# YangHai-1218/RADet

Measured on AMD Instinct MI355X. Metric: images/sec train-step, r50_ycbv_pbr 640x480 bs=4/GPU, higher is better.
Workload: dtype f32

## Files before the change

include/radet_hip.h:

```cpp
#ifndef RADET_HIP_H
#define RADET_HIP_H
#include <stdint.h>

#ifdef __cplusplus
extern "C" {
#endif


typedef struct RadetConvDesc {
    const float* w;
    const float* bias;
    const float* bn_gamma;
    const float* bn_beta;
    const float* bn_mean;
    const float* bn_var;
    float* wf;
    float* wft;
    float* bias_f;
    const float* dwf_slabs;
    const float* dbias_partials;
    float* dw;
    float* dbias;
    float* dgamma;
    float* dbeta;
// ... 192 lines not shown
                             void* yp1, float* stats1, float* partial_ws1, int B, int C, int groups, float eps, int relu,
                             const int* seg_desc, int nseg, void* stream);
int radet_gn_relu_bwd_p(const float* dy, const float* z, const float* stats, const float* gamma, const float* beta,
                        float* dz, void* dzp, float* dgamma, float* dbeta, float* partial_ws, int B, int C, int groups,
                        int relu, const int* seg_desc, int nseg, void* stream);
int radet_nchw_to_nhwc(const float* x, float* y, int B, int C, int H, int W, void* stream);
int radet_nhwc_to_nchw(const float* x, float* y, int B, int C, int H, int W, void* stream);

int radet_head_loss_ws_ints(int R);
int radet_head_loss(const float* cls, const float* reg_u, const float* iou, const float* scales,
                    const float* gt_boxes, const int64_t* gt_labels, const int* gt_off, const int64_t* p2g,
                    const float* pw, const int* level_desc, int nlvl, int B, int num_classes, float alpha,
                    float gamma, float loss_bbox_weight, float giou_eps, const float* grad_scale, float* losses,
                    float* dcls, int dcls_ld, float* dreg_u, int dreg_ld, float* diou, int diou_ld, float* dscales,
                    int64_t* labels_out, float* bbox_targets_out, int flags, int* ws, void* stream);
int radet_scale_relu(const float* reg_u, const float* scales, float* out, const int* level_desc, int nlvl, int B,
                     void* stream);

size_t radet_decode_ws_bytes(int B, int nlvl, int nms_pre);
int radet_decode_candidates(const float* cls, const float* reg_u, const float* iou, const float* scales,
                            const int* level_desc, int nlvl, int B, int num_classes, float score_thr, int nms_pre,
                            const float* img_hw , const float* scale_factor ,
                            float* cand_boxes, float* cand_scores, float* cand_ctr, int64_t* cand_labels,
                            int* cand_count, void* ws, void* stream);

size_t radet_nms_ws_bytes(int B, int cap);
int radet_nms(const float* boxes, const float* cluster_scores, const float* vote_scores, const int64_t* labels,
              const int* counts, int B, int cap, int mode, float iou_thr, int iou_enable, float sigma, int max_out,
              float* out_boxes, float* out_scores, int64_t* out_labels, int* out_count, int64_t* aux0, int64_t* aux1,
              void* ws, void* stream);
// ... 169 lines not shown
```

radet_amd/_lib.py:

```python
import ctypes as C
import os

_HERE = os.path.dirname(os.path.abspath(__file__))
LIB_PATH = os.path.join(_HERE, os.environ.get("RADET_LIB", "libradet_hip.so"))

_p = C.c_void_p
_i = C.c_int
_f = C.c_float
_sz = C.c_size_t


class RadetConvDesc(C.Structure):
    _fields_ = [("w", _p), ("bias", _p), ("bn_gamma", _p), ("bn_beta", _p), ("bn_mean", _p), ("bn_var", _p),
                ("wf", _p), ("wft", _p), ("bias_f", _p), ("dwf_slabs", _p), ("dbias_partials", _p),
                ("dw", _p), ("dbias", _p), ("dgamma", _p), ("dbeta", _p),
                ("cout", _i), ("cin", _i), ("kh", _i), ("kw", _i), ("nsplit", _i), ("eps", _f),
                ("wft_ld", _i), ("wft_off", _i), ("w16", _i), ("w_amax", _p), ("wfq", _p), ("w_l1", _p), ("bias_amax", _p),
                ("w_l1t", _p)]


class RadetScales(C.Structure):
    _fields_ = [("x_amax", _p), ("w_amax", _p), ("y_amax", _p), ("x1_amax", _p), ("w1_amax", _p), ("y1_amax", _p),
                ("yq", _p), ("yq_amax", _p), ("x_true_amax", _p), ("w_l1", _p), ("bias_amax", _p), ("addend_amax", _p)]

# ... 45 lines not shown
    "radet_stem_wgrad": (_i, [_p, _p, _p, _p, _i, _i, _i, _i, _p]),
    "radet_gn_workspace_floats": (_i, [_i, _p, _i]),
    "radet_gn_relu_fwd": (_i, [_p, _p, _p, _p, _p, _p, _i, _i, _i, _f, _i, _p, _i, _p]),
    "radet_gn_relu_fwd_pair": (_i, [_p] * 12 + [_i, _i, _i, _f, _i, _p, _i, _p]),
    "radet_gn_relu_fwd_pair_h": (_i, [_p] * 12 + [_i, _i, _i, _f, _i, _p, _i, _p]),
    "radet_gn_relu_bwd": (_i, [_p, _p, _p, _p, _p, _p, _p, _p, _p, _i, _i, _i, _i, _p, _i, _p]),
    "radet_upsample_add": (_i, [_p, _p, _i, _i, _i, _i, _i, _i, _p]),
    "radet_upsample_add_bwd": (_i, [_p, _p, _i, _i, _i, _i, _i, _i, _p]),
    "radet_relu_bwd": (_i, [_p, _p, _p, _p, _sz, _p]),
    "radet_nchw_to_nhwc": (_i, [_p, _p, _i, _i, _i, _i, _p]),
    "radet_nhwc_to_nchw": (_i, [_p, _p, _i, _i, _i, _i, _p]),
    "radet_head_loss_ws_ints": (_i, [_i]),
    "radet_head_loss": (_i, [_p, _p, _p, _p, _p, _p, _p, _p, _p, _p, _i, _i, _i, _f, _f, _f, _f, _p, _p, _p, _i, _p,
                             _i, _p, _i, _p, _p, _p, _i, _p, _p]),
    "radet_scale_relu": (_i, [_p, _p, _p, _p, _i, _i, _p]),
    "radet_decode_ws_bytes": (_sz, [_i, _i, _i]),
    "radet_decode_candidates": (_i, [_p, _p, _p, _p, _p, _i, _i, _i, _f, _i, _p, _p, _p, _p, _p, _p, _p, _p, _p]),
    "radet_nms_ws_bytes": (_sz, [_i, _i]),
    "radet_nms": (_i, [_p, _p, _p, _p, _p, _i, _i, _i, _f, _i, _f, _i, _p, _p, _p, _p, _p, _p, _p, _p]),
    "radet_assign_ws_bytes": (_sz, [_i, _i]),
    "radet_assign_points": (_i, [_p, _p, _p, _i, _i, _p, _i, _p, _p, _i, _i, _i, _i, _f, _p, _p, _p, _p, _p]),
    "radet_assign_points_f": (_i, [_p, _p, _p, _i, _i, _p, _i, _p, _p, _i, _i, _i, _i, _f, _p, _p, _p, _p, _p]),
    "radet_resize_linear_u8": (_i, [_p, _p, _p, _p, _i, _i, _i, _p]),
    "radet_resize_linear_u8_window": (_i, [_p, _p, _p, _p, _i, _i, _i, _p]),
    "radet_resize_linear_u8_src_window": (_i, [_p, _p, _p, _p, _i, _i, _i, _p]),
    "radet_resize_linear_f": (_i, [_p, _p, _p, _p, _i, _i, _i, _p]),
    "radet_warp_affine_u8": (_i, [_p, _sz, _p, _sz, _p, _i, _i, _i, _p]),
    "radet_gaussian_blur9_u8": (_i, [_p, _p, _p, _p, _p, _i, _i, _p]),
    "radet_sobel_edge": (_i, [_p, _p, _p, _p, _p, _i, _i, _p]),
    "radet_stem_conv_bn_relu_h": (_i, [_p, _p, _p, _p, _i, _i, _i, _p]),
# ... 108 lines not shown
```

radet_amd/csrc/tape_thunks.c:

```c
#include <stdint.h>
#include <stddef.h>
#include <string.h>
#include "radet_hip.h"

static float f32(uint64_t w) { uint32_t u = (uint32_t)w; float f; memcpy(&f, &u, 4); return f; }

static int t_radet_absmax(const uint64_t* a) { return radet_absmax((void*)(uintptr_t)a[0], (size_t)a[1], (void*)(uintptr_t)a[2], (void*)(uintptr_t)a[3]); }
static int t_radet_adamw_step(const uint64_t* a) { return radet_adamw_step((void*)(uintptr_t)a[0], (void*)(uintptr_t)a[1], (void*)(uintptr_t)a[2], (void*)(uintptr_t)a[3], (size_t)a[4], f32(a[5]), f32(a[6]), f32(a[7]), f32(a[8]), f32(a[9]), (int)(int64_t)a[10], f32(a[11]), f32(a[12]), (void*)(uintptr_t)a[13], (int)(int64_t)a[14], (void*)(uintptr_t)a[15], (void*)(uintptr_t)a[16]); }
static int t_radet_amax_slot_words(const uint64_t* a) { (void)a; return radet_amax_slot_words(); }
static int t_radet_assign_points(const uint64_t* a) { return radet_assign_points((void*)(uintptr_t)a[0], (void*)(uintptr_t)a[1], (void*)(uintptr_t)a[2], (int)(int64_t)a[3], (int)(int64_t)a[4], (void*)(uintptr_t)a[5], (int)(int64_t)a[6], (void*)(uintptr_t)a[7], (void*)(uintptr_t)a[8], (int)(int64_t)a[9], (int)(int64_t)a[10], (int)(int64_t)a[11], (int)(int64_t)a[12], f32(a[13]), (void*)(uintptr_t)a[14], (void*)(uintptr_t)a[15], (void*)(uintptr_t)a[16], (void*)(uintptr_t)a[17], (void*)(uintptr_t)a[18]); }
static int t_radet_assign_points_f(const uint64_t* a) { return radet_assign_points_f((void*)(uintptr_t)a[0], (void*)(uintptr_t)a[1], (void*)(uintptr_t)a[2], (int)(int64_t)a[3], (int)(int64_t)a[4], (void*)(uintptr_t)a[5], (int)(int64_t)a[6], (void*)(uintptr_t)a[7], (void*)(uintptr_t)a[8], (int)(int64_t)a[9], (int)(int64_t)a[10], (int)(int64_t)a[11], (int)(int64_t)a[12], f32(a[13]), (void*)(uintptr_t)a[14], (void*)(uintptr_t)a[15], (void*)(uintptr_t)a[16], (void*)(uintptr_t)a[17], (void*)(uintptr_t)a[18]); }
static int t_radet_augment_box(const uint64_t* a) { return radet_augment_box((void*)(uintptr_t)a[0], (void*)(uintptr_t)a[1], (void*)(uintptr_t)a[2], (size_t)a[3], (int)(int64_t)a[4], (int)(int64_t)a[5], (int)(int64_t)a[6], (void*)(uintptr_t)a[7]); }
static int t_radet_augment_finish(const uint64_t* a) { return radet_augment_finish((void*)(uintptr_t)a[0], (void*)(uintptr_t)a[1], (void*)(uintptr_t)a[2], (void*)(uintptr_t)a[3], (int)(int64_t)a[4], (int)(int64_t)a[5], (int)(int64_t)a[6], f32(a[7]), f32(a[8]), f32(a[9]), f32(a[10]), f32(a[11]), f32(a[12]), (void*)(uintptr_t)a[13]); }
static int t_radet_augment_hsv_noise(const uint64_t* a) { return radet_augment_hsv_noise((void*)(uintptr_t)a[0], (void*)(uintptr_t)a[1], (void*)(uintptr_t)a[2], (int)(int64_t)a[3], (int)(int64_t)a[4], (void*)(uintptr_t)a[5]); }
static int t_radet_augment_merge_hblur(const uint64_t* a) { return radet_augment_merge_hblur((void*)(uintptr_t)a[0], (void*)(uintptr_t)a[1], (void*)(uintptr_t)a[2], (void*)(uintptr_t)a[3], (int)(int64_t)a[4], (int)(int64_t)a[5], (int)(int64_t)a[6], (void*)(uintptr_t)a[7]); }
static int t_radet_augment_sharp(const uint64_t* a) { return radet_augment_sharp((void*)(uintptr_t)a[0], (void*)(uintptr_t)a[1], (void*)(uintptr_t)a[2], (void*)(uintptr_t)a[3], (int)(int64_t)a[4], (int)(int64_t)a[5], (void*)(uintptr_t)a[6]); }
static int t_radet_augment_vblur(const uint64_t* a) { return radet_augment_vblur((void*)(uintptr_t)a[0], (void*)(uintptr_t)a[1], (void*)(uintptr_t)a[2], (int)(int64_t)a[3], (int)(int64_t)a[4], (int)(int64_t)a[5], (void*)(uintptr_t)a[6]); }
static int t_radet_bbox_overlaps(const uint64_t* a) { return radet_bbox_overlaps((void*)(uintptr_t)a[0], (void*)(uintptr_t)a[1], (void*)(uintptr_t)a[2], (int)(int64_t)a[3], (int)(int64_t)a[4], (int)(int64_t)a[5], (int)(int64_t)a[6], (int)(int64_t)a[7], f32(a[8]), (void*)(uintptr_t)a[9]); }
static int t_radet_bce_logits_loss(const uint64_t* a) { return radet_bce_logits_loss((void*)(uintptr_t)a[0], (void*)(uintptr_t)a[1], (void*)(uintptr_t)a[2], (int)(int64_t)a[3], (size_t)a[4], (int)(int64_t)a[5], (void*)(uintptr_t)a[6], f32(a[7]), (void*)(uintptr_t)a[8], (void*)(uintptr_t)a[9]); }
static int t_radet_bce_logits_loss_bwd(const uint64_t* a) { return radet_bce_logits_loss_bwd((void*)(uintptr_t)a[0], (void*)(uintptr_t)a[1], (void*)(uintptr_t)a[2], (int)(int64_t)a[3], (size_t)a[4], (int)(int64_t)a[5], (void*)(uintptr_t)a[6], (void*)(uintptr_t)a[7], (void*)(uintptr_t)a[8], f32(a[9]), (void*)(uintptr_t)a[10], (void*)(uintptr_t)a[11]); }
static int t_radet_build_gather_table(const uint64_t* a) { return radet_build_gather_table((void*)(uintptr_t)a[0], (int)(int64_t)a[1], (int)(int64_t)a[2], (int)(int64_t)a[3], (int)(int64_t)a[4], (int)(int64_t)a[5], (int)(int64_t)a[6], (int)(int64_t)a[7], (void*)(uintptr_t)a[8], (int)(int64_t)a[9], (void*)(uintptr_t)a[10]); }
static int t_radet_coco_accumulate(const uint64_t* a) { return radet_coco_accumulate((void*)(uintptr_t)a[0], (void*)(uintptr_t)a[1], (void*)(uintptr_t)a[2], (void*)(uintptr_t)a[3], (void*)(uintptr_t)a[4], (void*)(uintptr_t)a[5], (void*)(uintptr_t)a[6], (void*)(uintptr_t)a[7], (int)(int64_t)a[8], (int)(int64_t)a[9], (int)(int64_t)a[10], (int)(int64_t)a[11], (int)(int64_t)a[12], (void*)(uintptr_t)a[13], (void*)(uintptr_t)a[14], (void*)(uintptr_t)a[15], (void*)(uintptr_t)a[16]); }
static int t_radet_coco_match(const uint64_t* a) { return radet_coco_match((void*)(uintptr_t)a[0], (void*)(uintptr_t)a[1], (void*)(uintptr_t)a[2], (void*)(uintptr_t)a[3], (void*)(uintptr_t)a[4], (void*)(uintptr_t)a[5], (int)(int64_t)a[6], (int)(int64_t)a[7], (void*)(uintptr_t)a[8], (int)(int64_t)a[9], (void*)(uintptr_t)a[10], (int)(int64_t)a[11], (void*)(uintptr_t)a[12], (void*)(uintptr_t)a[13], (void*)(uintptr_t)a[14], (void*)(uintptr_t)a[15], (void*)(uintptr_t)a[16]); }
static int t_radet_conv2d_igemm(const uint64_t* a) { return radet_conv2d_igemm((void*)(uintptr_t)a[0], (void*)(uintptr_t)a[1], (void*)(uintptr_t)a[2], (void*)(uintptr_t)a[3], (void*)(uintptr_t)a[4], (void*)(uintptr_t)a[5], (void*)(uintptr_t)a[6], (int)(int64_t)a[7], (int)(int64_t)a[8], (int)(int64_t)a[9], (int)(int64_t)a[10], (int)(int64_t)a[11], (int)(int64_t)a[12], (int)(int64_t)a[13], (void*)(uintptr_t)a[14], (size_t)a[15], (void*)(uintptr_t)a[16]); }
// ... 45 lines not shown
static int t_radet_mask_transform_src_window(const uint64_t* a) { return radet_mask_transform_src_window((void*)(uintptr_t)a[0], (void*)(uintptr_t)a[1], (void*)(uintptr_t)a[2], (void*)(uintptr_t)a[3], (int)(int64_t)a[4], (int)(int64_t)a[5], (int)(int64_t)a[6], (int)(int64_t)a[7], (int)(int64_t)a[8], (int)(int64_t)a[9], (void*)(uintptr_t)a[10]); }
static int t_radet_mask_transform_window(const uint64_t* a) { return radet_mask_transform_window((void*)(uintptr_t)a[0], (void*)(uintptr_t)a[1], (void*)(uintptr_t)a[2], (void*)(uintptr_t)a[3], (int)(int64_t)a[4], (int)(int64_t)a[5], (int)(int64_t)a[6], (int)(int64_t)a[7], (int)(int64_t)a[8], (int)(int64_t)a[9], (void*)(uintptr_t)a[10]); }
static int t_radet_maxpool3x3s2(const uint64_t* a) { return radet_maxpool3x3s2((void*)(uintptr_t)a[0], (void*)(uintptr_t)a[1], (int)(int64_t)a[2], (int)(int64_t)a[3], (int)(int64_t)a[4], (int)(int64_t)a[5], (void*)(uintptr_t)a[6]); }
static int t_radet_maxpool3x3s2_a(const uint64_t* a) { return radet_maxpool3x3s2_a((void*)(uintptr_t)a[0], (void*)(uintptr_t)a[1], (int)(int64_t)a[2], (int)(int64_t)a[3], (int)(int64_t)a[4], (int)(int64_t)a[5], (void*)(uintptr_t)a[6], (void*)(uintptr_t)a[7]); }
static int t_radet_maxpool3x3s2_bwd_relu(const uint64_t* a) { return radet_maxpool3x3s2_bwd_relu((void*)(uintptr_t)a[0], (void*)(uintptr_t)a[1], (void*)(uintptr_t)a[2], (int)(int64_t)a[3], (int)(int64_t)a[4], (int)(int64_t)a[5], (int)(int64_t)a[6], (void*)(uintptr_t)a[7]); }
static int t_radet_maxpool3x3s2_h(const uint64_t* a) { return radet_maxpool3x3s2_h((void*)(uintptr_t)a[0], (void*)(uintptr_t)a[1], (int)(int64_t)a[2], (int)(int64_t)a[3], (int)(int64_t)a[4], (int)(int64_t)a[5], (void*)(uintptr_t)a[6]); }
static int t_radet_maxpool3x3s2_q(const uint64_t* a) { return radet_maxpool3x3s2_q((void*)(uintptr_t)a[0], (void*)(uintptr_t)a[1], (int)(int64_t)a[2], (int)(int64_t)a[3], (int)(int64_t)a[4], (int)(int64_t)a[5], (void*)(uintptr_t)a[6], (void*)(uintptr_t)a[7], (void*)(uintptr_t)a[8], (void*)(uintptr_t)a[9], (void*)(uintptr_t)a[10]); }
static int t_radet_mbd(const uint64_t* a) { return radet_mbd((void*)(uintptr_t)a[0], (void*)(uintptr_t)a[1], (int)(int64_t)a[2], (void*)(uintptr_t)a[3], (void*)(uintptr_t)a[4], f32(a[5]), (int)(int64_t)a[6], (int)(int64_t)a[7], (void*)(uintptr_t)a[8], (size_t)a[9], (void*)(uintptr_t)a[10], (void*)(uintptr_t)a[11]); }
static int t_radet_merge_pairs(const uint64_t* a) { return radet_merge_pairs((void*)(uintptr_t)a[0], (void*)(uintptr_t)a[1], (size_t)a[2], (int)(int64_t)a[3], (int)(int64_t)a[4], (void*)(uintptr_t)a[5], (void*)(uintptr_t)a[6]); }
static int t_radet_merge_planes(const uint64_t* a) { return radet_merge_planes((void*)(uintptr_t)a[0], (void*)(uintptr_t)a[1], (size_t)a[2], (int)(int64_t)a[3], (int)(int64_t)a[4], (void*)(uintptr_t)a[5]); }
static int t_radet_nchw_to_nhwc(const uint64_t* a) { return radet_nchw_to_nhwc((void*)(uintptr_t)a[0], (void*)(uintptr_t)a[1], (int)(int64_t)a[2], (int)(int64_t)a[3], (int)(int64_t)a[4], (int)(int64_t)a[5], (void*)(uintptr_t)a[6]); }
static int t_radet_nhwc_to_nchw(const uint64_t* a) { return radet_nhwc_to_nchw((void*)(uintptr_t)a[0], (void*)(uintptr_t)a[1], (int)(int64_t)a[2], (int)(int64_t)a[3], (int)(int64_t)a[4], (int)(int64_t)a[5], (void*)(uintptr_t)a[6]); }
static int t_radet_nms(const uint64_t* a) { return radet_nms((void*)(uintptr_t)a[0], (void*)(uintptr_t)a[1], (void*)(uintptr_t)a[2], (void*)(uintptr_t)a[3], (void*)(uintptr_t)a[4], (int)(int64_t)a[5], (int)(int64_t)a[6], (int)(int64_t)a[7], f32(a[8]), (int)(int64_t)a[9], f32(a[10]), (int)(int64_t)a[11], (void*)(uintptr_t)a[12], (void*)(uintptr_t)a[13], (void*)(uintptr_t)a[14], (void*)(uintptr_t)a[15], (void*)(uintptr_t)a[16], (void*)(uintptr_t)a[17], (void*)(uintptr_t)a[18], (void*)(uintptr_t)a[19]); }
static int t_radet_paste_maps(const uint64_t* a) { return radet_paste_maps((void*)(uintptr_t)a[0], (size_t)a[1], (int)(int64_t)a[2], (void*)(uintptr_t)a[3], (int)(int64_t)a[4], (int)(int64_t)a[5], (int)(int64_t)a[6], (void*)(uintptr_t)a[7], (void*)(uintptr_t)a[8]); }
static int t_radet_pred3x3_patch(const uint64_t* a) { return radet_pred3x3_patch((void*)(uintptr_t)a[0], (int)(int64_t)a[1], (void*)(uintptr_t)a[2], (int)(int64_t)a[3], (void*)(uintptr_t)a[4], (void*)(uintptr_t)a[5], (void*)(uintptr_t)a[6], (int)(int64_t)a[7], (void*)(uintptr_t)a[8], (void*)(uintptr_t)a[9], (void*)(uintptr_t)a[10], (int)(int64_t)a[11], (void*)(uintptr_t)a[12]); }
static int t_radet_preprocess_frames(const uint64_t* a) { return radet_preprocess_frames((void*)(uintptr_t)a[0], (int)(int64_t)a[1], (int)(int64_t)a[2], (int)(int64_t)a[3], f32(a[4]), f32(a[5]), f32(a[6]), f32(a[7]), f32(a[8]), f32(a[9]), (void*)(uintptr_t)a[10], (void*)(uintptr_t)a[11]); }
static int t_radet_relu_bwd(const uint64_t* a) { return radet_relu_bwd((void*)(uintptr_t)a[0], (void*)(uintptr_t)a[1], (void*)(uintptr_t)a[2], (void*)(uintptr_t)a[3], (size_t)a[4], (void*)(uintptr_t)a[5]); }
static int t_radet_relu_bwd_a(const uint64_t* a) { return radet_relu_bwd_a((void*)(uintptr_t)a[0], (void*)(uintptr_t)a[1], (void*)(uintptr_t)a[2], (void*)(uintptr_t)a[3], (size_t)a[4], (void*)(uintptr_t)a[5], (void*)(uintptr_t)a[6]); }
static int t_radet_relu_bwd_h(const uint64_t* a) { return radet_relu_bwd_h((void*)(uintptr_t)a[0], (void*)(uintptr_t)a[1], (void*)(uintptr_t)a[2], (void*)(uintptr_t)a[3], (size_t)a[4], (void*)(uintptr_t)a[5]); }
static int t_radet_resize_linear_f(const uint64_t* a) { return radet_resize_linear_f((void*)(uintptr_t)a[0], (void*)(uintptr_t)a[1], (void*)(uintptr_t)a[2], (void*)(uintptr_t)a[3], (int)(int64_t)a[4], (int)(int64_t)a[5], (int)(int64_t)a[6], (void*)(uintptr_t)a[7]); }
static int t_radet_resize_linear_u8(const uint64_t* a) { return radet_resize_linear_u8((void*)(uintptr_t)a[0], (void*)(uintptr_t)a[1], (void*)(uintptr_t)a[2], (void*)(uintptr_t)a[3], (int)(int64_t)a[4], (int)(int64_t)a[5], (int)(int64_t)a[6], (void*)(uintptr_t)a[7]); }
static int t_radet_resize_linear_u8_src_window(const uint64_t* a) { return radet_resize_linear_u8_src_window((void*)(uintptr_t)a[0], (void*)(uintptr_t)a[1], (void*)(uintptr_t)a[2], (void*)(uintptr_t)a[3], (int)(int64_t)a[4], (int)(int64_t)a[5], (int)(int64_t)a[6], (void*)(uintptr_t)a[7]); }
static int t_radet_resize_linear_u8_window(const uint64_t* a) { return radet_resize_linear_u8_window((void*)(uintptr_t)a[0], (void*)(uintptr_t)a[1], (void*)(uintptr_t)a[2], (void*)(uintptr_t)a[3], (int)(int64_t)a[4], (int)(int64_t)a[5], (int)(int64_t)a[6], (void*)(uintptr_t)a[7]); }
static int t_radet_rle_masks(const uint64_t* a) { return radet_rle_masks((void*)(uintptr_t)a[0], (int)(int64_t)a[1], (void*)(uintptr_t)a[2], (int)(int64_t)a[3], (void*)(uintptr_t)a[4], (int)(int64_t)a[5], (void*)(uintptr_t)a[6], (void*)(uintptr_t)a[7], (int)(int64_t)a[8], (int)(int64_t)a[9], (int)(int64_t)a[10], (int)(int64_t)a[11], (int)(int64_t)a[12], (void*)(uintptr_t)a[13]); }
static int t_radet_rle_masks_src_window(const uint64_t* a) { return radet_rle_masks_src_window((void*)(uintptr_t)a[0], (int)(int64_t)a[1], (void*)(uintptr_t)a[2], (int)(int64_t)a[3], (void*)(uintptr_t)a[4], (void*)(uintptr_t)a[5], (int)(int64_t)a[6], (void*)(uintptr_t)a[7], (void*)(uintptr_t)a[8], (int)(int64_t)a[9], (int)(int64_t)a[10], (int)(int64_t)a[11], (void*)(uintptr_t)a[12]); }
static int t_radet_rle_masks_window(const uint64_t* a) { return radet_rle_masks_window((void*)(uintptr_t)a[0], (int)(int64_t)a[1], (void*)(uintptr_t)a[2], (int)(int64_t)a[3], (void*)(uintptr_t)a[4], (void*)(uintptr_t)a[5], (int)(int64_t)a[6], (void*)(uintptr_t)a[7], (void*)(uintptr_t)a[8], (int)(int64_t)a[9], (int)(int64_t)a[10], (int)(int64_t)a[11], (void*)(uintptr_t)a[12]); }
static int t_radet_scale_relu(const uint64_t* a) { return radet_scale_relu((void*)(uintptr_t)a[0], (void*)(uintptr_t)a[1], (void*)(uintptr_t)a[2], (void*)(uintptr_t)a[3], (int)(int64_t)a[4], (int)(int64_t)a[5], (void*)(uintptr_t)a[6]); }
static int t_radet_sigmoid_focal_loss(const uint64_t* a) { return radet_sigmoid_focal_loss((void*)(uintptr_t)a[0], (void*)(uintptr_t)a[1], (void*)(uintptr_t)a[2], (int)(int64_t)a[3], (size_t)a[4], (int)(int64_t)a[5], f32(a[6]), f32(a[7]), (void*)(uintptr_t)a[8], f32(a[9]), (void*)(uintptr_t)a[10], (void*)(uintptr_t)a[11]); }
static int t_radet_sigmoid_focal_loss_bwd(const uint64_t* a) { return radet_sigmoid_focal_loss_bwd((void*)(uintptr_t)a[0], (void*)(uintptr_t)a[1], (void*)(uintptr_t)a[2], (int)(int64_t)a[3], (size_t)a[4], (int)(int64_t)a[5], f32(a[6]), f32(a[7]), (void*)(uintptr_t)a[8], (void*)(uintptr_t)a[9], (void*)(uintptr_t)a[10], f32(a[11]), (void*)(uintptr_t)a[12], (void*)(uintptr_t)a[13]); }
static int t_radet_sobel_edge(const uint64_t* a) { return radet_sobel_edge((void*)(uintptr_t)a[0], (void*)(uintptr_t)a[1], (void*)(uintptr_t)a[2], (void*)(uintptr_t)a[3], (void*)(uintptr_t)a[4], (int)(int64_t)a[5], (int)(int64_t)a[6], (void*)(uintptr_t)a[7]); }
// ... 86 lines not shown
    {"radet_mask_transform_src_window", t_radet_mask_transform_src_window, 11},
    {"radet_mask_transform_window", t_radet_mask_transform_window, 11},
    {"radet_maxpool3x3s2", t_radet_maxpool3x3s2, 7},
    {"radet_maxpool3x3s2_a", t_radet_maxpool3x3s2_a, 8},
    {"radet_maxpool3x3s2_bwd_relu", t_radet_maxpool3x3s2_bwd_relu, 8},
    {"radet_maxpool3x3s2_h", t_radet_maxpool3x3s2_h, 7},
    {"radet_maxpool3x3s2_q", t_radet_maxpool3x3s2_q, 11},
    {"radet_mbd", t_radet_mbd, 12},
    {"radet_merge_pairs", t_radet_merge_pairs, 7},
    {"radet_merge_planes", t_radet_merge_planes, 6},
    {"radet_nchw_to_nhwc", t_radet_nchw_to_nhwc, 7},
    {"radet_nhwc_to_nchw", t_radet_nhwc_to_nchw, 7},
    {"radet_nms", t_radet_nms, 20},
    {"radet_paste_maps", t_radet_paste_maps, 9},
    {"radet_pred3x3_patch", t_radet_pred3x3_patch, 13},
    {"radet_preprocess_frames", t_radet_preprocess_frames, 12},
    {"radet_relu_bwd", t_radet_relu_bwd, 6},
    {"radet_relu_bwd_a", t_radet_relu_bwd_a, 7},
    {"radet_relu_bwd_h", t_radet_relu_bwd_h, 6},
    {"radet_resize_linear_f", t_radet_resize_linear_f, 8},
    {"radet_resize_linear_u8", t_radet_resize_linear_u8, 8},
    {"radet_resize_linear_u8_src_window", t_radet_resize_linear_u8_src_window, 8},
    {"radet_resize_linear_u8_window", t_radet_resize_linear_u8_window, 8},
    {"radet_rle_masks", t_radet_rle_masks, 14},
    {"radet_rle_masks_src_window", t_radet_rle_masks_src_window, 13},
    {"radet_rle_masks_window", t_radet_rle_masks_window, 13},
    {"radet_scale_relu", t_radet_scale_relu, 7},
    {"radet_sigmoid_focal_loss", t_radet_sigmoid_focal_loss, 12},
    {"radet_sigmoid_focal_loss_bwd", t_radet_sigmoid_focal_loss_bwd, 14},
    {"radet_sobel_edge", t_radet_sobel_edge, 8},
// ... 6 lines not shown
    {"radet_stem_wgrad", t_radet_stem_wgrad, 9},
    {"radet_stem_wgrad_splits", t_radet_stem_wgrad_splits, 3},
    {"radet_stream_create_cumask", t_radet_stream_create_cumask, 3},
    {"radet_tblr_decode", t_radet_tblr_decode, 10},
    {"radet_tblr_encode", t_radet_tblr_encode, 7},
    {"radet_threshold_compact", t_radet_threshold_compact, 6},
    {"radet_unfold_grads", t_radet_unfold_grads, 4},
    {"radet_upsample_add", t_radet_upsample_add, 9},
    {"radet_upsample_add_a", t_radet_upsample_add_a, 10},
    {"radet_upsample_add_bwd", t_radet_upsample_add_bwd, 9},
    {"radet_upsample_add_bwd_a", t_radet_upsample_add_bwd_a, 10},
    {"radet_upsample_add_bwd_h", t_radet_upsample_add_bwd_h, 9},
    {"radet_upsample_add_h", t_radet_upsample_add_h, 9},
    {"radet_warp_affine_u8", t_radet_warp_affine_u8, 9},
};
const int radet_tape_nthunks = 113;
```

radet_amd/engine.py:

```python
import contextlib
import ctypes as C
import os

import torch

from . import _lib
from . import kernels as K
from .kernels import ConvGeom, Levels

ARCH = {50: (3, 4, 6, 3), 101: (3, 4, 23, 3)}


def conv_out_hw(h, w, k, s, p):
    return (h + 2 * p - k) // s + 1, (w + 2 * p - k) // s + 1


class _StemSplits:

    def __init__(self, nsplit):
        self.nsplit = nsplit


class Conv:

# ... 19 lines not shown
        self._watched = {}
        self.math = 1 if math == "bf16" else 0
        self.h16 = math == "bf16-storage"
        x3mode = os.environ.get("RADET_X3", "h2")
        self.x3 = math == "fp32" and x3mode != "0"
        self.h2 = self.x3 and x3mode not in ("bf16", "b3")
        self.pairs = self.h2 and os.environ.get("RADET_PAIRS", "0") == "1"
        self.po = self.h2 and not self.pairs and os.environ.get("RADET_PAIRS_ONLY", "0") == "1"
        self.po_max_planes = int(os.environ.get("RADET_PAIRS_ONLY_MAX", "512"))
        self.pairs_from = int(os.environ.get("RADET_PAIRS_FROM", "2"))
        if self.x3 and "RADET_TOWER_MODE" not in os.environ:
            self.tower_mode = "pairbwd"
        self.p3 = self.x3 and self.tower_mode == "pairbwd" and feat % 32 == 0 and os.environ.get("RADET_P3", "1") != "0"
        self.math_name = math
        self.act_dtype = torch.bfloat16 if self.h16 else torch.float32
        self.p, self.g = params, grads
        self.depth, self.num_classes, self.frozen_stages = depth, num_classes, frozen_stages
        self.strides, self.stacked_convs, self.feat = tuple(strides), stacked_convs, feat
        self.dev = next(iter(params.values())).device
        self.convs = []
        self._build_layers()
        self._alloc_folded()
        self.geo_key = None
        self.table = None

    TOWER_TAG = K.SYMBOL | K.BK32 | 3
    TOWER_TAG_FWD = K.SYMBOL | K.BK32 | 2

    tower_stages = K.STAGES3 if os.environ.get("RADET_TOWER_STAGES3", "0") == "1" else 0
    tower_tile = int(os.environ.get("RADET_TOWER_TILE", "6"))
# ... 300 lines not shown
                    self.buf[f"{t}.zhat{i}"] = slot(aux=True)
                self.buf[f"{t}.stats{i}"] = torch.empty(len(hw) * B * 64, device=dev)
            new(f"{t}.dy", R, f)
            for nm in (f"{t}.dz0", f"{t}.dz1"):
                if self.p3:
                    self.buf[nm] = K.Planes(R, f, device=dev, kind=pkind)
                else:
                    new(nm, R, f)
            self.buf[f"{t}.dz"] = self.buf[f"{t}.dz0"]
        for c in self.cls_tower + self.reg_tower:
            c.geom = ConvGeom(self.plv, f, f, 3, 1, 1)
            if self.p3 and self.h2:
                c.geom.nsplit = max(1, min(64, 256 // (-(-f // 128) * (f // 32)), (R + 127) // 128))
        for c in (self.pred_cls, self.pred_reg, self.pred_iou):
            c.geom = ConvGeom(self.plv, f, c.cout, 3, 1, 1)
        new("cls", R, self.num_classes, torch.float32)
        new("reg_u", R, 4, torch.float32)
        new("iou", R, 1, torch.float32)
        self.buf["dcls"] = torch.zeros(R, self.cls_pad, device=dev)
        self.buf["dregiou"] = torch.zeros(R, 16, device=dev)
        if self.h2:
            for nm in ("dcls", "dregiou"):
                self._amax_keys.append(K.register_amax(self.buf[nm], slot(), by_storage=True))
        if self.h16:
            self.buf["dcls16"] = torch.zeros(R, self.cls_pad, device=dev, dtype=torch.bfloat16)
            self.buf["dregiou16"] = torch.zeros(R, self.ri_pad, device=dev, dtype=torch.bfloat16)
        self.gn_ws = torch.empty(K.gn_ws_floats(self.plv), device=dev)
        self.gn_ws2 = torch.empty(K.gn_ws_floats(self.plv), device=dev)
        self.ldesc, self.nlvl = K.level_desc(self.plv, self.strides)
        self.loss_ws = torch.zeros(K.head_loss_ws_ints(R), dtype=torch.int32, device=dev)
# ... 614 lines not shown
        ts = [self.p[n] for n in names]
        base = ts[0].data_ptr()
        if all(t.data_ptr() == base + 4 * i for i, t in enumerate(ts)):
            return torch.as_strided(ts[0], (len(ts),), (1,))
        return torch.stack([t.reshape(()) for t in ts]).contiguous()

    def loss(self, gt_boxes, gt_labels, gt_off, p2g, pw, grad_scale=None, alpha=0.25, gamma=2.0, lbw=2.0,
             labels_out=None, tgt_out=None):
        b = self.buf
        dri = b["dregiou"]
        K.head_loss(b["cls"], b["reg_u"], b["iou"], self.scales_tensor(), gt_boxes, gt_labels, gt_off, p2g, pw, self.ldesc,
                    self.nlvl, self.B, self.num_classes, alpha, gamma, lbw, 1e-6, grad_scale, self.losses, b["dcls"],
                    self.cls_pad, dri, 16, dri.view(-1)[4:], 16, self.dscales, self.loss_ws, labels_out, tgt_out)
        if self.h2:
            K.absmax(b["dcls"], K.amax_slot(b["dcls"]))
            K.absmax(dri, K.amax_slot(dri))
        if self.h16:
            K.convert_rows(b["dcls"], b["dcls16"])
            K.convert_rows(dri, b["dregiou16"], ncols=4)
            K.convert_rows(dri, b["dregiou16"], ncols=1, src_off=4, dst_off=self.iou_col)
        return self.losses

    def _head_grads(self):
        b = self.buf
        return (b["dcls16"], b["dregiou16"]) if self.h16 else (b["dcls"], b["dregiou"])

    def _tower_bwd_head(self, t):
        b = self.buf
        ylast = b[f"{t}.y{self.stacked_convs - 1}"]
        dy = b[f"{t}.dy"]
        dcls, dri = self._head_grads()
        if t == "cls":
            pc = self.pred_cls
            K.conv_wgrad(pc.geom, dcls, ylast, pc.slabs, pc.dbias_partials, cout=pc.cout, ld_dy=self.cls_pad)
            K.conv_dgrad(pc.geom, dcls, pc.wft, dy, k_channels=self.cls_pad)
        else:
            pr, pi = self.pred_reg, self.pred_iou
            K.conv_wgrad(pr.geom, dri, ylast, pr.slabs, pr.dbias_partials, cout=4, ld_dy=self.ri_pad)
            K.conv_wgrad(pi.geom, dri.view(-1)[self.iou_col:], ylast, pi.slabs, pi.dbias_partials, cout=1, ld_dy=self.ri_pad)
            K.conv_dgrad(pr.geom, dri, pr.wft, dy, k_channels=self.ri_pad)

    def _tower_bwd_head_async(self, t):
        b = self.buf
        ylast = b[f"{t}.y{self.stacked_convs - 1}"]
        dy = b[f"{t}.dy"]
        side = self._side() if self.use_streams else None

        def wg(*a, **k):
            if side is None:
                K.conv_wgrad(*a, **k)
            else:
                self._fork(side)
                with torch.cuda.stream(side):
                    K.conv_wgrad(*a, **k)

        dcls, dri = self._head_grads()
        if t == "cls":
            pc = self.pred_cls
            wg(pc.geom, dcls, ylast, pc.slabs, pc.dbias_partials, cout=pc.cout, ld_dy=self.cls_pad)
            K.conv_dgrad(pc.geom, dcls, pc.wft, dy, k_channels=self.cls_pad)
        else:
            pr, pi = self.pred_reg, self.pred_iou
            wg(pr.geom, dri, ylast, pr.slabs, pr.dbias_partials, cout=4, ld_dy=self.ri_pad)
            wg(pi.geom, dri.view(-1)[self.iou_col:], ylast, pi.slabs, pi.dbias_partials, cout=1, ld_dy=self.ri_pad)
            K.conv_dgrad(pr.geom, dri, pr.wft, dy, k_channels=self.ri_pad)

    def _tower_bwd_layer(self, t, tower, i, ws, dP, addend):
        b, p, g = self.buf, self.p, self.g
        c = tower[i]
        dy, dz = b[f"{t}.dy"], b[f"{t}.dz"]
        gn = f"bbox_head.{t}_convs.{i}.gn"
        self._gn_bwd(dy, b[f"{t}.z{i}"], b[f"{t}.stats{i}"], p[gn + ".weight"], p[gn + ".bias"], dz,
                     g[gn + ".weight"], g[gn + ".bias"], ws)
        x = b[f"{t}.y{i - 1}"] if i > 0 else b["P"]
        K.conv_wgrad(c.geom, dz, x, c.slabs, None)
# ... 211 lines not shown
```

radet_amd/kernels.py:

```python
import ctypes as C
import os

import torch

from . import _lib

ID_MASK = 0xFF
SYMBOL = 0x100
BK32 = 0x200
MATH_BF16 = 0x400
STORE_BF16, OUT_F32 = 0x800, 0x10000
SPLITK, SPLITK_MASK = 0x1000, 0xF000
STAGES3 = 0x20000
STAGES4 = 0x40000
ROWPAIRS = 0x80000
STREAMK, STREAMK_MASK = 0x100000, 0x700000
X3 = 0x1000000
P3 = 0x2000000
H2 = 0x8000000
MASKQ = 0x10000000
WG_MATH_BF16, WG_STORE_BF16 = 0x1, 0x2
WG_TILE, WG_TILE_MASK = 0x10, 0x30
WG_ONE_TAP = 0x40
WG_PX32 = 0x80
# ... 955 lines not shown
                      g.nsplit_pairs or g.nsplit, fl, _stream(), _scales(dy, x, None))
            return
        _lib.call("radet_conv2d_wgrad", _ptr(dy.t), _ptr(x.t), _ptr(slabs), _ptr(dbias_partials), _ptr(g.fwd_table), g.lout.rows,
                  g.cin, co, co if ld_dy is None else ld_dy, g.k, g.k, g.nsplit, WG_P3 | (g.wgrad_flags & WG_ONE_TAP), _stream())
        return
    if getattr(g, "h2", False) and getattr(g, "x3", False) and not g.math and not _is16(dy):
        _lib.call("radet_conv2d_wgrad_s", _ptr(dy), _ptr(x), _ptr(slabs), _ptr(dbias_partials), _ptr(g.fwd_table), g.lout.rows,
                  g.cin, co, co if ld_dy is None else ld_dy, g.k, g.k, g.nsplit, WG_H2 | WG_ONE_TAP | g.wgrad_flags, _stream(),
                  _scales(dy, x, None))
        return
    _lib.call("radet_conv2d_wgrad", _ptr(dy), _ptr(x), _ptr(slabs), _ptr(dbias_partials), _ptr(g.fwd_table), g.lout.rows,
              g.cin, co, co if ld_dy is None else ld_dy, g.k, g.k, g.nsplit,
              (WG_STORE_BF16 if _is16(dy) else (WG_MATH_BF16 if g.math else (WG_X3 if getattr(g, "x3", False) else 0))) | g.wgrad_flags, _stream())


def conv_wgrad_group(jobs, tile=128, math=0):
    jobs = sorted(jobs, key=lambda j: -(j["g"].lout.rows // j["g"].nsplit))
    for i in range(0, len(jobs), 32):
        part = jobs[i:i + 32]
        arr = (_lib.RadetWgradJob * len(part))()
        for a, j in zip(arr, part):
            g = j["g"]
            a.dy, a.x, a.slabs = _ptr(j["dy"]), _ptr(j["x"]), _ptr(j["slabs"])
            a.dbias_partials, a.gather_table = _ptr(j.get("dbias")), _ptr(g.fwd_table)
            a.M, a.Cin, a.Cout, a.ld_dy, a.KH, a.KW, a.S = g.lout.rows, g.cin, g.cout, g.cout, g.k, g.k, g.nsplit
        _lib.call("radet_conv2d_wgrad_group", arr, len(part), (WG_MATH_BF16 if math else 0) | (1 if tile == 128 else 2) * WG_TILE, _stream())


def group_splits(geoms, tile=128, slots=512):
    best = None
# ... 648 lines not shown
```

Baseline: 504.5.

## Exploit sparse regression/IoU gradients in pred head backward

Adds sparse wgrad and dgrad kernels for the reg/IoU prediction convs. Wgrad visits only the positive rows listed by the loss workspace, and dgrad skips output tiles whose incoming gradients are all zero. Both replace dense GEMM-style conv backward calls that mostly multiplied zeros. The change also drops the separate absmax pass over the reg/IoU gradient and fixes the split count for these convs. It relies on the loss kernel emitting a correct positive-row list and count, and on gradients being zero at every other row.

```diff
diff --git a/include/radet_hip.h b/include/radet_hip.h
--- a/include/radet_hip.h
+++ b/include/radet_hip.h
@@ -230,6 +230,11 @@
                     float gamma, float loss_bbox_weight, float giou_eps, const float* grad_scale, float* losses,
                     float* dcls, int dcls_ld, float* dreg_u, int dreg_ld, float* diou, int diou_ld, float* dscales,
                     int64_t* labels_out, float* bbox_targets_out, int flags, int* ws, void* stream);
+int radet_pred_sparse_wgrad(const int* rows, const int* count, const float* dregiou, int ld, const void* x,
+                            const void* x_amax, const int* gather_table, int M, int Cin, int S, float* slabs_reg,
+                            float* dbias_reg, float* slabs_iou, float* dbias_iou, void* stream);
+int radet_pred_sparse_dgrad(const float* dregiou, int ld, const float* wf_reg, const float* wf_iou,
+                            const int* gather_table, int M, int Cin, float* dy, void* dy_amax, void* stream);
 int radet_scale_relu(const float* reg_u, const float* scales, float* out, const int* level_desc, int nlvl, int B,
                      void* stream);
 
diff --git a/radet_amd/_lib.py b/radet_amd/_lib.py
--- a/radet_amd/_lib.py
+++ b/radet_amd/_lib.py
@@ -83,6 +83,8 @@
     "radet_head_loss": (_i, [_p, _p, _p, _p, _p, _p, _p, _p, _p, _p, _i, _i, _i, _f, _f, _f, _f, _p, _p, _p, _i, _p,
                              _i, _p, _i, _p, _p, _p, _i, _p, _p]),
     "radet_scale_relu": (_i, [_p, _p, _p, _p, _i, _i, _p]),
+    "radet_pred_sparse_wgrad": (_i, [_p, _p, _p, _i, _p, _p, _p, _i, _i, _i, _p, _p, _p, _p, _p]),
+    "radet_pred_sparse_dgrad": (_i, [_p, _i, _p, _p, _p, _i, _i, _p, _p, _p]),
     "radet_decode_ws_bytes": (_sz, [_i, _i, _i]),
     "radet_decode_candidates": (_i, [_p, _p, _p, _p, _p, _i, _i, _i, _f, _i, _p, _p, _p, _p, _p, _p, _p, _p, _p]),
     "radet_nms_ws_bytes": (_sz, [_i, _i]),
diff --git a/radet_amd/csrc/pred_sparse.hip b/radet_amd/csrc/pred_sparse.hip
--- /dev/null
+++ b/radet_amd/csrc/pred_sparse.hip
@@ -0,0 +1,198 @@
+#include "common.h"
+#include "../../include/radet_hip.h"
+
+#define PS_BATCH 64
+#define PS_NG 5
+
+template <bool PAIRS>
+__global__ __launch_bounds__(256) void pred_sparse_wgrad_kernel(const int* __restrict__ rows, const int* __restrict__ count,
+                                                                const float* __restrict__ dri, int ld,
+                                                                const void* __restrict__ xv_, const unsigned* __restrict__ x_amax,
+                                                                const int* __restrict__ tab, int M, int Mp, int Cin,
+                                                                float* __restrict__ slabs_reg, float* __restrict__ dbias_reg,
+                                                                float* __restrict__ slabs_iou, float* __restrict__ dbias_iou) {
+    const int s = blockIdx.x, S = gridDim.x, t = blockIdx.y;
+    const int tid = threadIdx.x, c = blockIdx.z * 256 + tid;
+    float inv = 1.f;
+    if (PAIRS) inv = radet_pow2(-radet_h2_exp(radet_amax_read(x_amax)));
+    int P = count[0];
+    P = P < 0 ? 0 : (P > M ? M : P);
+    const int per = (P + S - 1) / S;
+    const int k0 = min(s * per, P), k1 = min(k0 + per, P);
+    __shared__ int ssrc[PS_BATCH];
+    __shared__ float sg[PS_BATCH][8];
+    const bool bias_thread = t == 0 && blockIdx.z == 0 && tid < PS_NG;
+    const bool live = c < Cin;
+    const int cc = live ? c : 0;
+    float acc[PS_NG] = {0.f, 0.f, 0.f, 0.f, 0.f};
+    float bsum = 0.f;
+    for (int kb = k0; kb < k1; kb += PS_BATCH) {
+        const int n = min(PS_BATCH, k1 - kb);
+        __syncthreads();
+        if (tid < PS_BATCH) {
+            int src = -1;
+            float4 g = make_float4(0.f, 0.f, 0.f, 0.f);
+            float g4 = 0.f;
+            if (tid < n) {
+                const int m = rows[kb + tid];
+                if ((unsigned)m < (unsigned)M) {
+                    src = tab[(size_t)t * Mp + m];
+                    if ((unsigned)src >= (unsigned)M) src = -1;
+                    g = *reinterpret_cast<const float4*>(dri + (size_t)m * ld);
+                    g4 = dri[(size_t)m * ld + 4];
+                }
+            }
+            ssrc[tid] = src;
+            sg[tid][0] = g.x; sg[tid][1] = g.y; sg[tid][2] = g.z; sg[tid][3] = g.w; sg[tid][4] = g4;
+        }
+        __syncthreads();
+        for (int j = 0; j < n; j += 8) {
+            float xv[8];
+#pragma unroll
+            for (int u = 0; u < 8; ++u) {
+                const int src = ssrc[j + u];
+                float v = 0.f;
+                if (src >= 0) {
+                    if (PAIRS) {
+                        const unsigned short* p = reinterpret_cast<const unsigned short*>(xv_) + (size_t)src * 2 * Cin + radet_pair_off(cc);
+                        v = radet_pair_value(p[0], p[32]) * inv;
+                    } else {
+                        v = reinterpret_cast<const float*>(xv_)[(size_t)src * Cin + cc];
+                    }
+                }
+                xv[u] = v;
+            }
+#pragma unroll
+            for (int u = 0; u < 8; ++u)
+#pragma unroll
+                for (int o = 0; o < PS_NG; ++o) acc[o] = fmaf(sg[j + u][o], xv[u], acc[o]);
+        }
+        if (bias_thread)
+            for (int j = 0; j < n; ++j) bsum += sg[j][tid];
+    }
+    if (live) {
+#pragma unroll
+        for (int o = 0; o < 4; ++o) slabs_reg[(((size_t)s * 4 + o) * 9 + t) * Cin + c] = acc[o];
+        slabs_iou[((size_t)s * 9 + t) * Cin + c] = acc[4];
+    }
+    if (bias_thread) {
+        if (tid < 4) dbias_reg[s * 4 + tid] = bsum;
+        else dbias_iou[s] = bsum;
+    }
+}
+
+#define PD_ROWS 64
+
+__global__ __launch_bounds__(256) void pred_sparse_dgrad_kernel(const float* __restrict__ dri, int ld,
+                                                                const float* __restrict__ wf_reg, const float* __restrict__ wf_iou,
+                                                                const int* __restrict__ tab, int M, int Mp, int Cin,
+                                                                float* __restrict__ dy, unsigned* __restrict__ dy_amax) {
+    __shared__ float4 sw[9 * PS_NG * 64];
+    __shared__ float sg[9][PD_ROWS][PS_NG];
+    __shared__ int snz[9][PD_ROWS];
+    __shared__ int slist[PD_ROWS];
+    __shared__ int snnz;
+    const int tid = threadIdx.x, lane = tid & 63, wave = tid >> 6;
+    const int m0 = blockIdx.x * PD_ROWS, C4 = Cin >> 2;
+    constexpr int NP = (9 * PD_ROWS + 255) / 256;
+    int q[NP];
+#pragma unroll
+    for (int u = 0; u < NP; ++u) {
+        const int i = tid + 256 * u, t = i >> 6, m = m0 + (i & 63);
+        q[u] = (t < 9 && m < M) ? tab[(size_t)t * Mp + m] : -1;
+    }
+    float4* dy4 = reinterpret_cast<float4*>(dy);
+    for (int rl = wave * (PD_ROWS / 4); rl < (wave + 1) * (PD_ROWS / 4); ++rl) {
+        const int m = m0 + rl;
+        if (m < M)
+            for (int c4 = lane; c4 < C4; c4 += 64) dy4[(size_t)m * C4 + c4] = make_float4(0.f, 0.f, 0.f, 0.f);
+    }
+    float4 ga[NP];
+    float gb[NP];
+#pragma unroll
+    for (int u = 0; u < NP; ++u) {
+        const bool ok = (unsigned)q[u] < (unsigned)M;
+        const size_t o = ok ? (size_t)q[u] * ld : 0;
+        ga[u] = *reinterpret_cast<const float4*>(dri + o);
+        gb[u] = dri[o + 4];
+        if (!ok) { ga[u] = make_float4(0.f, 0.f, 0.f, 0.f); gb[u] = 0.f; }
+    }
+#pragma unroll
+    for (int u = 0; u < NP; ++u) {
+        const int i = tid + 256 * u, t = i >> 6, rl = i & 63;
+        if (t < 9) {
+            const float4 a = ga[u];
+            snz[t][rl] = (a.x != 0.f || a.y != 0.f || a.z != 0.f || a.w != 0.f || gb[u] != 0.f) ? 1 : 0;
+            sg[t][rl][0] = a.x; sg[t][rl][1] = a.y; sg[t][rl][2] = a.z; sg[t][rl][3] = a.w; sg[t][rl][4] = gb[u];
+        }
+    }
+    __syncthreads();
+    if (wave == 0) {
+        bool nz = false;
+#pragma unroll
+        for (int t = 0; t < 9; ++t) nz = nz || snz[t][lane] != 0;
+        const unsigned long long bal = __ballot(nz);
+        if (nz) slist[__popcll(bal & ((1ull << lane) - 1ull))] = lane;
+        if (lane == 0) snnz = __popcll(bal);
+    }
+    __syncthreads();
+    const int nnz = snnz;
+    float am = 0.f;
+    if (nnz > 0) {
+        for (int i = tid; i < 9 * PS_NG * C4; i += 256) {
+            const int to = i / C4, c4 = i - to * C4;
+            const int t = to / PS_NG, o = to - t * PS_NG;
+            const float* w = o < 4 ? wf_reg + ((size_t)o * 9 + t) * Cin : wf_iou + (size_t)t * Cin;
+            sw[to * 64 + c4] = reinterpret_cast<const float4*>(w)[c4];
+        }
+        __syncthreads();
+        if (lane < C4) {
+            for (int k = wave; k < nnz; k += 4) {
+                const int rl = slist[k];
+                float4 acc = make_float4(0.f, 0.f, 0.f, 0.f);
+#pragma unroll
+                for (int t = 0; t < 9; ++t) {
+                    if (!snz[t][rl]) continue;
+#pragma unroll
+                    for (int o = 0; o < PS_NG; ++o) {
+                        const float g = sg[t][rl][o];
+                        const float4 w = sw[(t * PS_NG + o) * 64 + lane];
+                        acc.x = fmaf(g, w.x, acc.x);
+                        acc.y = fmaf(g, w.y, acc.y);
+                        acc.z = fmaf(g, w.z, acc.z);
+                        acc.w = fmaf(g, w.w, acc.w);
+                    }
+                }
+                dy4[(size_t)(m0 + rl) * C4 + lane] = acc;
+                am = fmaxf(fmaxf(am, fmaxf(fabsf(acc.x), fabsf(acc.y))), fmaxf(fabsf(acc.z), fabsf(acc.w)));
+            }
+        }
+    }
+    if (dy_amax) radet_amax_publish(am, dy_amax);
+}
+
+extern "C" int radet_pred_sparse_wgrad(const int* rows, const int* count, const float* dregiou, int ld, const void* x,
+                                       const void* x_amax, const int* gather_table, int M, int Cin, int S, float* slabs_reg,
+                                       float* dbias_reg, float* slabs_iou, float* dbias_iou, void* stream) {
+    if (!rows || !count || !dregiou || !x || !gather_table || !slabs_reg || !dbias_reg || !slabs_iou || !dbias_iou)
+        return RADET_ERR_ARG;
+    if (M <= 0 || Cin <= 0 || S < 1 || S > 65535 || ld < 8 || (ld & 3) || (x_amax && (Cin & 31))) return RADET_ERR_ARG;
+    const dim3 grid(S, 9, (Cin + 255) / 256);
+    const int Mp = radet_gather_table_rows(M);
+    if (x_amax)
+        hipLaunchKernelGGL(pred_sparse_wgrad_kernel<true>, grid, dim3(256), 0, (hipStream_t)stream, rows, count, dregiou, ld, x,
+                           (const unsigned*)x_amax, gather_table, M, Mp, Cin, slabs_reg, dbias_reg, slabs_iou, dbias_iou);
+    else
+        hipLaunchKernelGGL(pred_sparse_wgrad_kernel<false>, grid, dim3(256), 0, (hipStream_t)stream, rows, count, dregiou, ld, x,
+                           (const unsigned*)nullptr, gather_table, M, Mp, Cin, slabs_reg, dbias_reg, slabs_iou, dbias_iou);
+    return radet_check_launch();
+}
+
+extern "C" int radet_pred_sparse_dgrad(const float* dregiou, int ld, const float* wf_reg, const float* wf_iou,
+                                       const int* gather_table, int M, int Cin, float* dy, void* dy_amax, void* stream) {
+    if (!dregiou || !wf_reg || !wf_iou || !gather_table || !dy) return RADET_ERR_ARG;
+    if (M <= 0 || Cin <= 0 || Cin > 256 || (Cin & 3) || ld < 8 || (ld & 3)) return RADET_ERR_ARG;
+    hipLaunchKernelGGL(pred_sparse_dgrad_kernel, dim3((M + PD_ROWS - 1) / PD_ROWS), dim3(256), 0, (hipStream_t)stream, dregiou,
+                       ld, wf_reg, wf_iou, gather_table, M, radet_gather_table_rows(M), Cin, dy, (unsigned*)dy_amax);
+    return radet_check_launch();
+}
diff --git a/radet_amd/csrc/tape_thunks.c b/radet_amd/csrc/tape_thunks.c
--- a/radet_amd/csrc/tape_thunks.c
+++ b/radet_amd/csrc/tape_thunks.c
@@ -83,6 +83,8 @@
 static int t_radet_nms(const uint64_t* a) { return radet_nms((void*)(uintptr_t)a[0], (void*)(uintptr_t)a[1], (void*)(uintptr_t)a[2], (void*)(uintptr_t)a[3], (void*)(uintptr_t)a[4], (int)(int64_t)a[5], (int)(int64_t)a[6], (int)(int64_t)a[7], f32(a[8]), (int)(int64_t)a[9], f32(a[10]), (int)(int64_t)a[11], (void*)(uintptr_t)a[12], (void*)(uintptr_t)a[13], (void*)(uintptr_t)a[14], (void*)(uintptr_t)a[15], (void*)(uintptr_t)a[16], (void*)(uintptr_t)a[17], (void*)(uintptr_t)a[18], (void*)(uintptr_t)a[19]); }
 static int t_radet_paste_maps(const uint64_t* a) { return radet_paste_maps((void*)(uintptr_t)a[0], (size_t)a[1], (int)(int64_t)a[2], (void*)(uintptr_t)a[3], (int)(int64_t)a[4], (int)(int64_t)a[5], (int)(int64_t)a[6], (void*)(uintptr_t)a[7], (void*)(uintptr_t)a[8]); }
 static int t_radet_pred3x3_patch(const uint64_t* a) { return radet_pred3x3_patch((void*)(uintptr_t)a[0], (int)(int64_t)a[1], (void*)(uintptr_t)a[2], (int)(int64_t)a[3], (void*)(uintptr_t)a[4], (void*)(uintptr_t)a[5], (void*)(uintptr_t)a[6], (int)(int64_t)a[7], (void*)(uintptr_t)a[8], (void*)(uintptr_t)a[9], (void*)(uintptr_t)a[10], (int)(int64_t)a[11], (void*)(uintptr_t)a[12]); }
+static int t_radet_pred_sparse_dgrad(const uint64_t* a) { return radet_pred_sparse_dgrad((void*)(uintptr_t)a[0], (int)(int64_t)a[1], (void*)(uintptr_t)a[2], (void*)(uintptr_t)a[3], (void*)(uintptr_t)a[4], (int)(int64_t)a[5], (int)(int64_t)a[6], (void*)(uintptr_t)a[7], (void*)(uintptr_t)a[8], (void*)(uintptr_t)a[9]); }
+static int t_radet_pred_sparse_wgrad(const uint64_t* a) { return radet_pred_sparse_wgrad((void*)(uintptr_t)a[0], (void*)(uintptr_t)a[1], (void*)(uintptr_t)a[2], (int)(int64_t)a[3], (void*)(uintptr_t)a[4], (void*)(uintptr_t)a[5], (void*)(uintptr_t)a[6], (int)(int64_t)a[7], (int)(int64_t)a[8], (int)(int64_t)a[9], (void*)(uintptr_t)a[10], (void*)(uintptr_t)a[11], (void*)(uintptr_t)a[12], (void*)(uintptr_t)a[13], (void*)(uintptr_t)a[14]); }
 static int t_radet_preprocess_frames(const uint64_t* a) { return radet_preprocess_frames((void*)(uintptr_t)a[0], (int)(int64_t)a[1], (int)(int64_t)a[2], (int)(int64_t)a[3], f32(a[4]), f32(a[5]), f32(a[6]), f32(a[7]), f32(a[8]), f32(a[9]), (void*)(uintptr_t)a[10], (void*)(uintptr_t)a[11]); }
 static int t_radet_relu_bwd(const uint64_t* a) { return radet_relu_bwd((void*)(uintptr_t)a[0], (void*)(uintptr_t)a[1], (void*)(uintptr_t)a[2], (void*)(uintptr_t)a[3], (size_t)a[4], (void*)(uintptr_t)a[5]); }
 static int t_radet_relu_bwd_a(const uint64_t* a) { return radet_relu_bwd_a((void*)(uintptr_t)a[0], (void*)(uintptr_t)a[1], (void*)(uintptr_t)a[2], (void*)(uintptr_t)a[3], (size_t)a[4], (void*)(uintptr_t)a[5], (void*)(uintptr_t)a[6]); }
@@ -199,6 +201,8 @@
     {"radet_nms", t_radet_nms, 20},
     {"radet_paste_maps", t_radet_paste_maps, 9},
     {"radet_pred3x3_patch", t_radet_pred3x3_patch, 13},
+    {"radet_pred_sparse_dgrad", t_radet_pred_sparse_dgrad, 10},
+    {"radet_pred_sparse_wgrad", t_radet_pred_sparse_wgrad, 15},
     {"radet_preprocess_frames", t_radet_preprocess_frames, 12},
     {"radet_relu_bwd", t_radet_relu_bwd, 6},
     {"radet_relu_bwd_a", t_radet_relu_bwd_a, 7},
@@ -235,4 +239,4 @@
     {"radet_upsample_add_h", t_radet_upsample_add_h, 9},
     {"radet_warp_affine_u8", t_radet_warp_affine_u8, 9},
 };
-const int radet_tape_nthunks = 113;
+const int radet_tape_nthunks = 115;
diff --git a/radet_amd/engine.py b/radet_amd/engine.py
--- a/radet_amd/engine.py
+++ b/radet_amd/engine.py
@@ -57,6 +57,8 @@
         self.p3 = self.x3 and self.tower_mode == "pairbwd" and feat % 32 == 0 and os.environ.get("RADET_P3", "1") != "0"
         self.math_name = math
         self.act_dtype = torch.bfloat16 if self.h16 else torch.float32
+        self.pred_sparse = os.environ.get("RADET_PRED_SPARSE", "1") != "0" and not self.h16 and not (self.x3 and not self.h2) \
+            and feat % 4 == 0 and feat <= 256
         self.p, self.g = params, grads
         self.depth, self.num_classes, self.frozen_stages = depth, num_classes, frozen_stages
         self.strides, self.stacked_convs, self.feat = tuple(strides), stacked_convs, feat
@@ -387,6 +389,8 @@
                 c.geom.nsplit = max(1, min(64, 256 // (-(-f // 128) * (f // 32)), (R + 127) // 128))
         for c in (self.pred_cls, self.pred_reg, self.pred_iou):
             c.geom = ConvGeom(self.plv, f, c.cout, 3, 1, 1)
+        if self.pred_sparse:
+            self.pred_reg.geom.nsplit = self.pred_iou.geom.nsplit = K.PRED_SPARSE_SPLITS
         new("cls", R, self.num_classes, torch.float32)
         new("reg_u", R, 4, torch.float32)
         new("iou", R, 1, torch.float32)
@@ -1031,7 +1035,8 @@
                     self.cls_pad, dri, 16, dri.view(-1)[4:], 16, self.dscales, self.loss_ws, labels_out, tgt_out)
         if self.h2:
             K.absmax(b["dcls"], K.amax_slot(b["dcls"]))
-            K.absmax(dri, K.amax_slot(dri))
+            if not self.pred_sparse:
+                K.absmax(dri, K.amax_slot(dri))
         if self.h16:
             K.convert_rows(b["dcls"], b["dcls16"])
             K.convert_rows(dri, b["dregiou16"], ncols=4)
@@ -1041,6 +1046,11 @@
     def _head_grads(self):
         b = self.buf
         return (b["dcls16"], b["dregiou16"]) if self.h16 else (b["dcls"], b["dregiou"])
+
+    def _pred_sparse_wgrad(self, ylast):
+        pr, pi = self.pred_reg, self.pred_iou
+        K.pred_sparse_wgrad(pr.geom, self.loss_ws[16:], self.loss_ws[0:1], self.buf["dregiou"], ylast,
+                            (pr.slabs, pr.dbias_partials), (pi.slabs, pi.dbias_partials))
 
     def _tower_bwd_head(self, t):
         b = self.buf
@@ -1051,6 +1061,9 @@
             pc = self.pred_cls
             K.conv_wgrad(pc.geom, dcls, ylast, pc.slabs, pc.dbias_partials, cout=pc.cout, ld_dy=self.cls_pad)
             K.conv_dgrad(pc.geom, dcls, pc.wft, dy, k_channels=self.cls_pad)
+        elif self.pred_sparse:
+            self._pred_sparse_wgrad(ylast)
+            K.pred_sparse_dgrad(self.pred_reg.geom, dri, self.pred_reg.wf, self.pred_iou.wf, dy)
         else:
             pr, pi = self.pred_reg, self.pred_iou
             K.conv_wgrad(pr.geom, dri, ylast, pr.slabs, pr.dbias_partials, cout=4, ld_dy=self.ri_pad)
@@ -1076,6 +1089,14 @@
             pc = self.pred_cls
             wg(pc.geom, dcls, ylast, pc.slabs, pc.dbias_partials, cout=pc.cout, ld_dy=self.cls_pad)
             K.conv_dgrad(pc.geom, dcls, pc.wft, dy, k_channels=self.cls_pad)
+        elif self.pred_sparse:
+            if side is None:
+                self._pred_sparse_wgrad(ylast)
+            else:
+                self._fork(side)
+                with torch.cuda.stream(side):
+                    self._pred_sparse_wgrad(ylast)
+            K.pred_sparse_dgrad(self.pred_reg.geom, dri, self.pred_reg.wf, self.pred_iou.wf, dy)
         else:
             pr, pi = self.pred_reg, self.pred_iou
             wg(pr.geom, dri, ylast, pr.slabs, pr.dbias_partials, cout=4, ld_dy=self.ri_pad)
diff --git a/radet_amd/kernels.py b/radet_amd/kernels.py
--- a/radet_amd/kernels.py
+++ b/radet_amd/kernels.py
@@ -993,6 +993,26 @@
               (WG_STORE_BF16 if _is16(dy) else (WG_MATH_BF16 if g.math else (WG_X3 if getattr(g, "x3", False) else 0))) | g.wgrad_flags, _stream())
 
 
+PRED_SPARSE_SPLITS = 16
+
+
+def pred_sparse_wgrad(g, rows, count, dri, x, reg, iou):
+    assert dri.dtype == torch.float32 and dri.dim() == 2 and g.k == 3 and g.stride == 1 and g.pad == 1
+    assert not _isp(x) or x.kind == "h2"
+    S = g.nsplit
+    assert reg[0].numel() == S * 4 * 9 * g.cin and iou[0].numel() == S * 9 * g.cin and reg[1].numel() == S * 4 and iou[1].numel() == S
+    _lib.call("radet_pred_sparse_wgrad", _ptr(rows), _ptr(count), _ptr(dri), dri.stride(0), _ptr_any(x),
+              _ptr(x.amax) if _isp(x) else None, _ptr(g.fwd_table), g.lout.rows, g.cin, S, _ptr(reg[0]), _ptr(reg[1]),
+              _ptr(iou[0]), _ptr(iou[1]), _stream())
+
+
+def pred_sparse_dgrad(g, dri, wf_reg, wf_iou, dx):
+    assert dri.dtype == torch.float32 and dri.dim() == 2 and g.k == 3 and g.stride == 1 and g.pad == 1
+    assert wf_reg.dtype == torch.float32 and wf_iou.dtype == torch.float32 and dx.dtype == torch.float32
+    _lib.call("radet_pred_sparse_dgrad", _ptr(dri), dri.stride(0), _ptr(wf_reg), _ptr(wf_iou), _ptr(g.bwd_table), g.lin.rows,
+              g.cin, _ptr(dx), _ptr(amax_slot(dx)), _stream())
+
+
 def conv_wgrad_group(jobs, tile=128, math=0):
     jobs = sorted(jobs, key=lambda j: -(j["g"].lout.rows // j["g"].nsplit))
     for i in range(0, len(jobs), 32):
```

Result: no change. 507.5 (median of 6 runs) (+0.6%).
